# Kangfei/NNGP-src

Hardware: AMD Instinct MI355X
Metric: NNGP kernel-build + GP-solve wall-clock (ms) and GFLOP/s at N train queries (higher is better)
Workload: dtype f32 (Cholesky products as split f16 x3, f32 accumulate; f64 build/CG/means; the posterior's float64-grade residual as exact int8 digit-plane products); 1 GPU; synthetic N=32768, d=128, 5-layer ReLU NNGP + full Cholesky posterior (configs[2], north-star target); N=32768, d=128, n_relu=3, get=nngp, M_test=1024, parallelism=single GPU

## Files before the change

nngp-src_amd/csrc/api.hip:

```cpp
#include "model.h"

namespace nngp {

static thread_local char g_err[1024] = "";

void set_error(const char* fmt, ...) {
    va_list ap;
    va_start(ap, fmt);
    vsnprintf(g_err, sizeof(g_err), fmt, ap);
    va_end(ap);
}

int make_arch_dev(const nngp_arch* arch, ArchDev* out) {
    NNGP_REQUIRE(arch != nullptr, "arch is NULL");
    NNGP_REQUIRE(arch->n_dense >= 1 && arch->n_dense <= NNGP_MAX_DENSE, "arch.n_dense must be in [1, %d] (got %d)",
                 NNGP_MAX_DENSE, arch->n_dense);
    out->n_dense = arch->n_dense;
    out->groups = nullptr;
    for (int l = 0; l < NNGP_MAX_DENSE; ++l) {
        out->w2[l] = l < arch->n_dense ? arch->w_std[l] * arch->w_std[l] : 0.0;
        out->b2[l] = l < arch->n_dense ? arch->b_std[l] * arch->b_std[l] : 0.0;
    }
    return 0;
}
// ... 376 lines not shown
    NNGP_HIP_CHECK(hipStreamSynchronize(s));
    m->trace_mean = m->pcg.host_scal[7] / (double)n;
    m->diag_max = m->pcg.host_scal[6];
    m->reg = m->absolute ? m->diag_reg : m->diag_reg * m->trace_mean;
    m->reg_fac = m->reg;
    set_split_scale(m);
    m->have_train = true;
    return 0;
}

int nngp_model_build_rows(nngp_model* m, int64_t row_begin, int64_t row_end, void* stream) {
    hipStream_t s = (hipStream_t)stream;
    NNGP_REQUIRE(m != nullptr && m->have_train, "build_rows: call set_train first");
    NNGP_REQUIRE(0 <= row_begin && row_begin <= row_end && row_end <= m->n, "build_rows: bad row range");
    NNGP_TRY(drop_pending_solve(m));
    BuildArgs a{};
    a.x1 = m->x; a.x2 = m->x; a.q1 = m->q; a.q2 = m->q;
    a.n1 = m->n; a.n2 = m->n; a.d = m->d;
    a.row_begin = row_begin; a.row_end = row_end;
    a.sym = (row_begin == 0 && row_end == m->n) ? 1 : 0;
    a.ld64 = a.ld32 = m->ld;
    if (m->get == NNGP_GET_NNGP) a.nngp64 = m->k64; else a.ntk64 = m->k64;
    m->a32_built = false;
    m->a32_complete = false;
    m->k64_partial = false;
    m->k64_symmetric = a.sym != 0;
    m->i8.k.ready = false;
    m->i8_checked = m->i8_distrusted = false;
    m->i8_guard_pending = false;
    if (a.sym) {
// ... 10 lines not shown
        NNGP_TRY(launch_zero_pad_f64(m->kaux64, m->np, m->n, m->np, s));
        m->aux_ready = true;
        m->i8.aux.ready = false;
    }
    NNGP_TRY(launch_zero_pad_f64(m->k64, m->ld, m->n, m->np, s));
    m->built = true;
    m->factored = m->solved = false;
    m->solve_pending = false;
    return 0;
}

int nngp_model_factor_begin(nngp_model* m, void* stream) {
    hipStream_t s = (hipStream_t)stream;
    NNGP_REQUIRE(m != nullptr && m->built, "factor: build the kernel rows first");
    NNGP_TRY(drop_pending_solve(m));
    NNGP_TRY(launch_factor_input(m->k64, m->ld, m->a32, m->ld, m->n, m->np, m->reg_fac, m->reg_fac + m->trace_mean, s,
                                 m->a32_complete ? m->n : m->a32_built ? (m->n / TB) * TB : 0));
    m->a32_built = false;
    m->a32_complete = false;
    NNGP_HIP_CHECK(hipMemsetAsync(m->clamped, 0, sizeof(int32_t), s));
    m->tri.bs = triinv_block(m->np);
    m->factored = m->solved = false;
    m->solve_pending = false;
    m->serving_ready = false;
    m->split.l_ready = m->split.lt_ready = false;
    m->split.split_panel = -1;
    return 0;
}

int nngp_model_factor_panel(nngp_model* m, int64_t col0, int64_t width, void* stream) {
// ... 8 lines not shown
    return potrf_update_f32(m->a32, m->np, m->ld, panel_col0, panel_width, col0, width, (hipStream_t)stream, &m->split);
}

int nngp_model_factor_update_cols(nngp_model* m, int64_t panel_col0, int64_t panel_width, const int64_t* cols, int32_t ncols,
                                  int64_t width, void* stream) {
    NNGP_REQUIRE(m != nullptr && m->built, "factor_update_cols: build the kernel rows first");
    NNGP_REQUIRE(ncols >= 0 && (ncols == 0 || cols != nullptr), "factor_update_cols: bad column list");
    return potrf_update_cols_f32(m->a32, m->np, m->ld, panel_col0, panel_width, cols, ncols, width, (hipStream_t)stream, &m->split);
}

int nngp_model_factor_input_rows(nngp_model* m, int64_t row_begin, int64_t row_end, double shift_scale, void* stream) {
    hipStream_t s = (hipStream_t)stream;
    NNGP_REQUIRE(m != nullptr && m->built, "factor_input_rows: build the kernel rows first");
    NNGP_REQUIRE(0 <= row_begin && row_begin <= row_end && row_end <= m->n && shift_scale >= 1.0, "factor_input_rows: bad row range or shift");
    NNGP_TRY(drop_pending_solve(m));
    m->reg_fac = m->reg * shift_scale;
    m->k64_partial = true;
    return launch_factor_input(m->k64, m->ld, m->a32, m->ld, m->n, m->np, m->reg_fac, m->reg_fac + m->trace_mean, s, row_begin, row_end);
}

int nngp_model_factor_input_complete(nngp_model* m) {
    NNGP_REQUIRE(m != nullptr && m->built, "factor_input_complete: build the kernel rows first");
    NNGP_REQUIRE(m->k64_partial, "factor_input_complete: no rows of the factor input were converted (nngp_model_factor_input_rows) since the last build");
    m->a32_complete = true;
    return 0;
}

int nngp_model_precond(nngp_model* m, const double* r, double* z, void* stream) {
    NNGP_REQUIRE(m != nullptr && m->factored, "precond: factor first");
    NNGP_REQUIRE(r != nullptr && z != nullptr, "precond: NULL argument");
// ... 52 lines not shown
int nngp_model_factor(nngp_model* m, void* stream) {
    hipStream_t s = (hipStream_t)stream;
    NNGP_REQUIRE(m != nullptr && m->built, "factor: build the kernel rows first");
    if (!m->k64_partial) m->reg_fac = m->reg;
    set_split_scale(m);
    for (int attempt = 0;; ++attempt) {
        NNGP_TRY(nngp_model_factor_begin(m, stream));
        NNGP_TRY(potrf_lookahead_f32(m->a32, m->np, m->ld, m->dinv, m->clamped, (float)(0.25 * m->reg_fac), m->la, &m->split, s, &m->tri));
        int32_t cl = 0;
        NNGP_HIP_CHECK(hipMemcpyAsync(&cl, m->clamped, sizeof(int32_t), hipMemcpyDeviceToHost, s));
        NNGP_HIP_CHECK(hipStreamSynchronize(s));
        if (cl == 0 || attempt == 4 || NNGP_KNOB(6) == 1 || m->k64_partial) break;
        m->reg_fac *= 16.0;
        set_split_scale(m);
    }
    return nngp_model_factor_end(m, stream);
}

double nngp_model_factor_shift(nngp_model* m) { return m != nullptr ? m->reg_fac : 0.0; }

int nngp_model_append(nngp_model* m, const double* x_new, const double* y_new, int64_t b, void* stream) {
    hipStream_t s = (hipStream_t)stream;
    NNGP_REQUIRE(m != nullptr && m->factored, "append: fit the model first");
    NNGP_REQUIRE(!m->k64_partial, "append: not with the row-sharded layout (the model holds only its own kernel rows)");
    NNGP_REQUIRE(x_new != nullptr && y_new != nullptr && b > 0, "append: bad arguments");
    NNGP_REQUIRE(m->n + b <= m->n_cap, "append: %lld + %lld rows exceed n_cap = %lld", (long long)m->n, (long long)b,
                 (long long)m->n_cap);
    const int64_t n0 = m->n, n1 = n0 + b, np0 = m->np, np1 = round_up(n1, TB), r0 = (n0 / TB) * TB, rows = np1 - r0;
    NNGP_REQUIRE(r0 > 0, "append: the fitted model must have at least 128 rows");
    NNGP_TRY(drop_pending_solve(m));
    NNGP_TRY(ensure_predict_capacity(m, rows, false));
// ... 328 lines not shown
```

nngp-src_amd/csrc/api_predict.hip:

```cpp
#include "model.h"

namespace nngp {

int ensure_predict_capacity(nngp_model* m, int64_t mt, bool need_ktd) {
    if (mt > m->m_cap || m->b32 == nullptr) {
        const int64_t cap = mt > m->m_cap ? mt : m->m_cap;
        NNGP_HIP_CHECK(hipDeviceSynchronize());
        dev_free(m->xt_q); dev_free(m->tt_diag); dev_free(m->b32); dev_free(m->trsm_tmp);
        NNGP_TRY(dev_alloc(&m->xt_q, cap));
        NNGP_TRY(dev_alloc(&m->tt_diag, cap));
        NNGP_TRY(dev_alloc(&m->b32, round_up(cap, TB) * m->np_cap));
        NNGP_TRY(dev_alloc(&m->trsm_tmp, round_up(cap, TB) * triinv_block(m->np_cap)));
        if (m->split.planes != nullptr) {
            dev_free(m->split.planes_b); dev_free(m->split.row_inv);
            m->split.planes_b = nullptr; m->split.row_inv = nullptr;
            m->split.mb_cap = round_up(cap, TB);
            m->split.b_panels = (int)((triinv_block(m->np_cap) + m->split.k_cap - 1) / m->split.k_cap);
            NNGP_TRY(dev_alloc(&m->split.planes_b, (int64_t)(m->split.b_panels - 1) * m->split.col_stride + (m->split.mb_cap + 256) * m->split.k_cap * 4));
            NNGP_TRY(dev_alloc(&m->split.row_inv, m->split.mb_cap));
            tk_destroy(m->tk);
            m->tk = nullptr;
            if (m->split.k_cap == 1024 && triinv_block(m->np_cap) == 1024) NNGP_TRY(tk_create(&m->tk, m->np_cap, m->split.mb_cap) < 0 ? -1 : 0);
        }
        m->m_cap = cap;
// ... 169 lines not shown
int i8s_cut_planes(nngp_model* m, I8Planes& pk, const double* kmat, int64_t kld, hipStream_t s) {
    I8Work& w = m->i8;
    NNGP_TRY(launch_i8s_diag_bound_scale(kmat, kld, m->np, pk.scale, s));
    const bool sym = (kmat == m->kaux64 || m->k64_symmetric) && (pk.alloc_planes == 5 || pk.alloc_planes == 7) && NNGP_KNOB(5) != 62;
    if (sym)
        NNGP_TRY(launch_i8s_slice_sym(kmat, kld, m->np, pk.alloc_planes, pk.scale, pk.planes, m->np_cap, w.k_rows * m->np_cap, s));
    else
        NNGP_TRY(launch_i8s_slice_rows(kmat, kld, m->np, m->np, pk.alloc_planes, pk.scale, nullptr, pk.planes, m->np_cap, w.k_rows * m->np_cap, s));
    NNGP_TRY(launch_i8s_scale_sqsum(pk.scale, m->np, pk.scale + m->np_cap, s));
    pk.ns_done = pk.alloc_planes;
    pk.ready = true;
    return 0;
}

int i8s_product_rows(nngp_model* m, I8Planes& pk, const double* kmat, int64_t kld, double* out, const double* cin, double beta,
                     double alpha, double* z, double gamma, int64_t mp, hipStream_t s, int grade) {
    const int64_t np = m->np;
    I8Work& w = m->i8;
    const int fine_z = NNGP_KNOB(5) == 64 ? kI8FinePlanes : kI8FineZPlanes;
    const bool round_z = grade == I8_COARSE ? w.ns_z < w.ns_k : fine_z < kI8FinePlanes;
    const bool fuse_rows = grade == I8_COARSE && m->i8_fuse_request && cin != nullptr && w.rowpart_rows >= mp && NNGP_KNOB(5) != 59;
    const int ns_z = grade == I8_FINE ? fine_z : w.ns_z, ns_k = grade == I8_FINE ? kI8FinePlanes : w.ns_k;
    const int cut = grade == I8_FINE ? kI8FineCut : w.cut;
    NNGP_REQUIRE(pk.alloc_planes >= ns_k && w.z_planes >= ns_z, "i8s_product_rows: workspace for %d planes missing", ns_k);
    if (!pk.ready || pk.ns_done < ns_k) {
        NNGP_TRY(i8s_cut_planes(m, pk, kmat, kld, s));
    } else if (&pk == &m->i8.k && m->i8_k_pending) {
        NNGP_HIP_CHECK(hipStreamWaitEvent(s, m->ev_i8, 0));
    }
    if (&pk == &m->i8.k) m->i8_k_pending = false;
    I8Plan pl;
    NNGP_TRY(i8s_plan(ns_z, ns_k, cut, &pl));
    const int64_t nchunk = i8s_chunks(np, &pl);
    for (int64_t r0 = 0; r0 < mp; r0 += kI8RowBlock) {
        const int64_t mb = mp - r0 < kI8RowBlock ? mp - r0 : kI8RowBlock;
        const int64_t slab = mb * np;
        NNGP_TRY(launch_i8s_slice_rows(z + r0 * np, np, mb, np, ns_z, nullptr, w.zscale, w.zplanes, m->np_cap, (w.z_rows + 256) * m->np_cap, s,
                                       round_z ? z + r0 * np : nullptr));
        if (r0 == 0 && grade == I8_COARSE && !m->gate_recorded && NNGP_KNOB(2) != 8 && NNGP_KNOB(2) != 9 && !cg_from_the_start(m, mp)) {
            if (m->ev_gate == nullptr) NNGP_HIP_CHECK(hipEventCreateWithFlags(&m->ev_gate, hipEventDisableTiming));
            NNGP_HIP_CHECK(hipEventRecord(m->ev_gate, s));
            m->gate_recorded = true;
        }
        const bool timed = w.timed && w.t_count < I8Work::kMaxTimed;
        if (timed) {
            const int t = w.t_count;
            if (w.t0[t] == nullptr) NNGP_HIP_CHECK(hipEventCreate(&w.t0[t]));
            if (w.t1[t] == nullptr) NNGP_HIP_CHECK(hipEventCreate(&w.t1[t]));
            NNGP_HIP_CHECK(hipEventRecord(w.t0[t], s));
        }
        NNGP_TRY(launch_gemm_nt_i8s(w.partial, np, slab, w.zplanes, m->np_cap, (w.z_rows + 256) * m->np_cap, pk.planes, m->np_cap,
                                    w.k_rows * m->np_cap, pl, mb, np, np, w.counters, 0, s));
        if (timed) {
// ... 6 lines not shown
        fuse.out32 = m->b32 + r0 * np;
        fuse.ld32 = np;
        fuse.part = w.rowpart + r0 * i8s_col_blocks(np) * 4;
        NNGP_TRY(launch_i8s_combine(out + r0 * np, np, cin ? cin + r0 * np : nullptr, np, beta, alpha, z + r0 * np, np, gamma, w.partial, np,
                                    slab, (int)nchunk, pl.ndiag, w.zscale, pk.scale, mb, np, s, fuse_rows ? &fuse : nullptr));
    }
    if (fuse_rows) m->i8_fuse_done = true;
    if (grade == I8_COARSE && !m->gate_recorded && NNGP_KNOB(2) == 9) {
        if (m->ev_gate == nullptr) NNGP_HIP_CHECK(hipEventCreateWithFlags(&m->ev_gate, hipEventDisableTiming));
        NNGP_HIP_CHECK(hipEventRecord(m->ev_gate, s));
        m->gate_recorded = true;
    }
    return 0;
}

int residual_rows(nngp_model* m, double* out, const double* rhs, double* z, int64_t mp, hipStream_t s, bool first_residual) {
    const int64_t np = m->np;
    const bool coarse = first_residual;
    if (!coarse && use_i8s_fine(m, mp)) m->i8_want_fine = true;
    if (coarse ? use_i8s(m, mp) : use_i8s_fine(m, mp)) {
        const int rc = ensure_i8s(m, mp, m->i8.k, coarse ? i8s_planes_policy(m) : kI8FinePlanes);
        if (rc == 0) {
            if (coarse) m->i8_used_now = true;
            return i8s_product_rows(m, m->i8.k, m->k64, m->ld, out, rhs, 1.0, -1.0, z, -m->reg, mp, s, coarse ? I8_COARSE : I8_FINE);
        }
        if (rc != 1) return rc;
    }
    NNGP_TRY(launch_gemm_nt_f64(out, np, rhs, np, z, np, m->k64, m->ld, mp, np, np, -1.0, 1.0, s));
    return launch_axpby_mat(out, 1.0, z, -m->reg, np, mp, np, s);
}

int tri_join(nngp_model* m, hipStream_t s) {
    if (m->tri_stale) {
        if (m->ev_tri == nullptr) NNGP_HIP_CHECK(hipEventCreateWithFlags(&m->ev_tri, hipEventDisableTiming));
        NNGP_TRY(triinv_build(m->a32, m->ld, m->dinv, m->np, m->tri, s));
        if (m->tk != nullptr && m->tri.bs == 1024) NNGP_TRY(tk_prepare_inverses(m->tk, m->tri, m->np, m->a32, m->ld, s));
        NNGP_HIP_CHECK(hipEventRecord(m->ev_tri, s));
        m->tri_stale = false;
        m->tri_pending = true;
        return 0;
    }
    if (m->tri_pending) NNGP_HIP_CHECK(hipStreamWaitEvent(s, m->ev_tri, 0));
    if (m->tk != nullptr && !tk_inverses_ready(m->tk) && m->tri.bs == 1024) {
        NNGP_TRY(tk_prepare_inverses(m->tk, m->tri, m->np, m->a32, m->ld, s));
        if (m->ev_tri == nullptr) NNGP_HIP_CHECK(hipEventCreateWithFlags(&m->ev_tri, hipEventDisableTiming));
        NNGP_HIP_CHECK(hipEventRecord(m->ev_tri, s));
        m->tri_pending = true;
    }
    return 0;
}

int tri_fork(nngp_model* m, hipStream_t s) {
    if (!m->tri_stale || m->la == nullptr || m->la->panel == nullptr || NNGP_KNOB(5) == 61) return 0;
    if (m->ev_tri == nullptr) NNGP_HIP_CHECK(hipEventCreateWithFlags(&m->ev_tri, hipEventDisableTiming));
    if (m->ev_tri_fork == nullptr) NNGP_HIP_CHECK(hipEventCreateWithFlags(&m->ev_tri_fork, hipEventDisableTiming));
    NNGP_HIP_CHECK(hipEventRecord(m->ev_tri_fork, s));
    NNGP_HIP_CHECK(hipStreamWaitEvent(m->la->panel, m->ev_tri_fork, 0));
    NNGP_TRY(triinv_build(m->a32, m->ld, m->dinv, m->np, m->tri, m->la->panel));
    if (m->tk != nullptr && m->tri.bs == 1024) NNGP_TRY(tk_prepare_inverses(m->tk, m->tri, m->np, m->a32, m->ld, m->la->panel));
    NNGP_HIP_CHECK(hipEventRecord(m->ev_tri, m->la->panel));
    m->tri_stale = false;
    m->tri_pending = true;
    return 0;
}

bool use_split_solves(const nngp_model* m, int64_t mp) {
    return m->split.l_ready && m->split.planes_b != nullptr && mp <= m->split.mb_cap && m->tri.bs % m->split.k_cap == 0 &&
           m->tri.bs / m->split.k_cap <= m->split.b_panels && m->tri.bs <= 2048 && NNGP_KNOB(7) == 0 && mp >= 256 && mp * m->np >= 7000000;
}

bool use_tickets(const nngp_model* m, int64_t mp) {
    return !m->tk_failed && m->tri.bs == 1024 && tk_usable(m->tk, mp, m->np) && NNGP_KNOB(9) != 16;
}

bool cg_from_the_start(const nngp_model* m, int64_t mp) {
    static const int env = getenv("NNGP_TK_GATE") ? atoi(getenv("NNGP_TK_GATE")) : 1;
    return env != 0 && use_split_solves(m, mp) && use_tickets(m, mp);
// ... 77 lines not shown
    else NNGP_TRY(ensure_lt(m, s));
    int slot = -1;
    NNGP_TRY(trsm_timer_begin(m, mp, s, &slot));
    if (use_split_solves(m, mp) && use_tickets(m, mp))
        NNGP_TRY(tk_solve(m->tk, m->b32, m->np, mp, m->np, m->split, true, s, tickets_reserve(m)));
    else if (use_split_solves(m, mp))
        NNGP_TRY(trsm_rut_blocks_h3(m->b32, m->np, mp, m->lt_ready ? m->lt32 : nullptr, m->np, m->tri, m->np, m->trsm_tmp, m->split, s));
    else
        NNGP_TRY(trsm_rut_blocks_f32(m->b32, m->np, mp, m->lt32, m->np, m->tri, m->np, m->trsm_tmp, s));
    return trsm_timer_end(m, slot, s);
}

static int ntk_sweeps(const nngp_model* m) { return m->var_refine < 2 ? 2 : m->var_refine; }

int refined_solve_rows(nngp_model* m, const double* rhs, int64_t mp, int sweeps, bool final_residual, hipStream_t s,
                       bool measure) {
    const int64_t np = m->np;
    measure = measure && sweeps >= 2;
    NNGP_TRY(launch_convert_f64_f32(rhs, np, m->b32, np, mp, np, mp, np, s));
    NNGP_TRY(apply_inverse_f32(m, mp, s));
    NNGP_TRY(launch_f32_to_f64_mat(m->b32, np, m->z64, np, mp, np, false, s));
    for (int it = 0; it < sweeps + (final_residual ? 1 : 0); ++it) {
        NNGP_TRY(residual_rows(m, m->r64, rhs, m->z64, mp, s, it == 0));
        if (it == sweeps) break;
        NNGP_TRY(launch_convert_f64_f32(m->r64, np, m->b32, np, mp, np, mp, np, s));
        NNGP_TRY(apply_inverse_f32(m, mp, s));
        if (measure && it < 2) NNGP_TRY(launch_rows_energy(m->r64, m->b32, np, mp, np, it == 0 ? m->rows.var : m->rows.delta, s));
        NNGP_TRY(launch_f32_to_f64_mat(m->b32, np, m->z64, np, mp, np, true, s));
    }
    if (measure) NNGP_TRY(launch_rowdot_f64(m->z64, nullptr, 0.0, rhs, np, mp, np, nullptr, 1.0, m->rows.tol, s));
    return 0;
}

int rows_pcg_continue(nngp_model* m, int64_t mp, int max_iters, hipStream_t s) {
    const int64_t np = m->np;
    RowsPcg& w = m->rows;
    if (mp > m->rows_pq_cap) {
        NNGP_HIP_CHECK(hipDeviceSynchronize());
// ... 9 lines not shown
        NNGP_TRY(apply_inverse_f32(m, mp, s));
        NNGP_TRY(launch_rows_rho(m->r64, m->b32, np, mp, np, it == 0, w, s));
        NNGP_TRY(launch_rows_update_p(w.p, m->b32, np, mp, np, w, s));
        NNGP_TRY(launch_gemm_nt_f64(w.q, np, w.p, np, w.p, np, m->k64, m->ld, mp, np, np, 1.0, m->reg, s));
        NNGP_TRY(launch_rows_alpha(w.p, w.q, np, mp, np, w, s));
        NNGP_TRY(launch_rows_axpy2(m->z64, m->r64, w.p, w.q, np, mp, np, w, s));
        NNGP_HIP_CHECK(hipMemcpyAsync(w.host, w.live, sizeof(int32_t), hipMemcpyDeviceToHost, s));
        NNGP_HIP_CHECK(hipStreamSynchronize(s));
        m->cov_iters = it + 1;
        if (w.host[0] == 0) break;
    }
    return 0;
}

int build_cross(nngp_model* m, const double* xt, const double* qt, int64_t mt, int64_t mp, bool nngp, double* out,
                hipStream_t s) {
    NNGP_HIP_CHECK(hipMemsetAsync(out, 0, sizeof(double) * mp * m->np, s));
    BuildArgs a{};
    a.x1 = xt; a.x2 = m->x; a.q1 = qt; a.q2 = m->q;
    a.n1 = mt; a.n2 = m->n; a.d = m->d;
    a.row_begin = 0; a.row_end = mt; a.sym = 0;
    a.ld64 = a.ld32 = m->np;
    if (nngp) a.nngp64 = out; else a.ntk64 = out;
    return launch_kernel_build(a, m->arch, s);
}

}

extern "C" {

int nngp_model_prepare_serving(nngp_model* m, void* stream) {
    hipStream_t s = (hipStream_t)stream;
    NNGP_REQUIRE(m != nullptr && m->solved, "prepare_serving: fit the model first");
    NNGP_REQUIRE(!m->k64_partial, "prepare_serving: not with the row-sharded layout (the model holds only its own kernel rows)");
    if (m->get != NNGP_GET_NNGP) return 0;
    NNGP_TRY(run_pending_solve(m, s, true));
    const int64_t n = m->n, np = m->np;
    const int64_t blk = np < 1024 ? np : 1024;
// ... 61 lines not shown
            static const int cut_env = getenv("NNGP_TK_CUTSTREAM") ? atoi(getenv("NNGP_TK_CUTSTREAM")) : 2;
            hipStream_t cs = m->solve_stream;
            if (cut_env != 0 && cg_from_the_start(m, mp) && m->la != nullptr && m->la->panel != nullptr)
                cs = (cut_env == 2 && m->la->update != nullptr) ? m->la->update : m->la->panel;
            NNGP_HIP_CHECK(hipStreamWaitEvent(cs, m->ev_i8, 0));
            NNGP_TRY(i8s_cut_planes(m, m->i8.k, m->k64, m->ld, cs));
            NNGP_HIP_CHECK(hipEventRecord(m->ev_i8, cs));
            m->i8_k_pending = true;
        }
    }
    NNGP_TRY(tri_fork(m, s));

    const double* xt = on_train ? m->x : x_test;
    const double* ktd = m->k64;
    const double* qt = m->q;
    if (!on_train) {
        NNGP_TRY(launch_row_sqnorm(xt, mt, m->d, m->xt_q, s));
        qt = m->xt_q;
        NNGP_TRY(build_cross(m, xt, qt, mt, mp, !is_ntk, m->ktd64, s));
        ktd = m->ktd64;
    }
    if (compact_train) {
        NNGP_HIP_CHECK(hipMemsetAsync(m->ktd64, 0, sizeof(double) * mp * np, s));
        NNGP_HIP_CHECK(hipMemcpy2DAsync(m->ktd64, sizeof(double) * np, m->k64, sizeof(double) * m->ld, sizeof(double) * np, mt,
                                        hipMemcpyDeviceToDevice, s));
        ktd = m->ktd64;
    }
    if (m->i8_guard_pending && hipEventQuery(m->ev_guard) == hipSuccess) {
        double ratio = 0.0;
        memcpy(&ratio, m->i8_guard_host, sizeof(double));
        m->i8_guard_pending = false;
        if (ratio > m->i8_floor_ratio) m->i8_floor_ratio = ratio;
        if (!(ratio <= (NNGP_KNOB(5) == 56 ? 0.0 : kI8FloorThr))) m->i8_distrusted = true;
    }
    int check_kind = 0;
    bool i8_check_pending = false;
// ... 21 lines not shown
    const double kFlagThr = (NNGP_KNOB(6) >= 2 && NNGP_KNOB(6) <= 30) ? pow(10.0, -(double)NNGP_KNOB(6)) : 1e-8;
    auto cov_part = [&]() -> int {
    if (full) NNGP_TRY(ensure_full_cov_capacity(m, mt));
    NNGP_TRY(launch_kernel_diag(xt, qt, mt, m->d, m->arch, m->tt_diag, nullptr, s));
    auto build_ktt = [&]() -> int {
        BuildArgs a{};
        a.x1 = xt; a.x2 = xt; a.q1 = qt; a.q2 = qt;
        a.n1 = mt; a.n2 = mt; a.d = m->d;
        a.row_begin = 0; a.row_end = mt; a.sym = 1;
        a.ld64 = a.ld32 = mp;
        a.nngp64 = m->ktt64;
        return launch_kernel_build(a, m->arch, s);
    };

    if (!is_ntk && m->var_refine == 0) {
        NNGP_TRY(launch_convert_f64_f32(ktd, np, m->b32, np, mp, np, mp, np, s));
        NNGP_TRY(apply_forward_f32(m, mp, s));
        if (!full) return launch_row_sqsum_f32(m->b32, np, mt, np, m->tt_diag, var_or_cov, s);
        NNGP_TRY(build_ktt());
        NNGP_TRY(launch_gemm_nt_f32(m->vvt32, mp, m->b32, np, m->b32, np, mp, mp, np, 1.0f, 0.0f, false, s));
        return launch_cov_finish(m->ktt64, mp, m->vvt32, mp, mt, var_or_cov, s);
    }

    const bool serving = m->serving_ready && !is_ntk;
    if (!serving && !use_split_solves(m, mp)) NNGP_TRY(ensure_lt(m, s));
    NNGP_TRY(ensure_refine_capacity(m, mp));
    auto solve_rows = [&](int sweeps, bool final_residual) -> int {
        if (!serving) return refined_solve_rows(m, ktd, mp, sweeps, final_residual, s);
        NNGP_TRY(launch_gemm_nt_f64(m->z64, np, nullptr, 0, ktd, np, m->ainv64, np, mp, np, np, 1.0, 0.0, s));
        if (m->serving_weak) {
            NNGP_TRY(residual_rows(m, m->r64, ktd, m->z64, mp, s, false));
            NNGP_TRY(launch_gemm_nt_f64(m->z64, np, m->z64, np, m->r64, np, m->ainv64, np, mp, np, np, 1.0, 1.0, s));
        }
        if (final_residual) {
            NNGP_TRY(residual_rows(m, m->r64, ktd, m->z64, mp, s, false));
        }
        return 0;
    };
    if (!is_ntk) {
        const int level = ((serving || (full && m->var_refine == 1)) && m->var_refine < 2) ? 2 : m->var_refine;
        const bool second_order = level >= 2;
        if (!full && level == 1) {
            m->i8_fuse_request = true;
// ... 94 lines not shown
        NNGP_TRY(launch_zero_pad_f64(m->kaux64, np, n, np, s));
        m->aux_ready = true;
        m->i8.aux.ready = false;
    }
    const double* ktd_n = m->kaux64;
    if (!on_train) {
        if (mp > m->ktd_aux_cap) {
            NNGP_HIP_CHECK(hipDeviceSynchronize());
            dev_free(m->ktd_aux);
            NNGP_TRY(dev_alloc(&m->ktd_aux, mp * m->np_cap));
            m->ktd_aux_cap = mp;
        }
        NNGP_TRY(build_cross(m, xt, qt, mt, mp, true, m->ktd_aux, s));
        ktd_n = m->ktd_aux;
    }
    NNGP_TRY(refined_solve_rows(m, ktd, mp, ntk_sweeps(m), false, s, m->var_refine >= 1));
    ntk_cross = ktd_n;
    z_valid = true;
    if (full) NNGP_TRY(build_ktt());
    if (m->var_refine >= 1) check_kind = 3;
    NNGP_TRY(ntk_finish());
    if (check_kind == 3) {
        NNGP_TRY(launch_rows_dvar(m->b32, m->r64, full ? nullptr : ntk_cross, -1.0, np, mt, np, m->rows.coef, s));
        NNGP_TRY(launch_sweep_estimate(m->rows.var, m->rows.delta, m->rows.tol, m->rows.coef, var_or_cov, full ? mt + 1 : 1,
                                       mt, reinterpret_cast<double*>(m->rows.live + 2), s));
    }
    return 0;
    };
    if (cov_mode != NNGP_COV_NONE) NNGP_TRY(cov_part());
    NNGP_TRY(run_pending_solve(m, s, true, z_valid));
    if (i8_check_pending) {
// ... 81 lines not shown
```

nngp-src_amd/csrc/common.h:

```cpp
#pragma once
#include <hip/hip_runtime.h>
#include <stdint.h>
#include <atomic>
#include <stdio.h>
#include <string.h>

#include "../../include/nngp_hip.h"
#include "../../include/nngp_rbf_gp.h"
#include "../../include/nngp_activations.h"
#include "../../include/nngp_mll.h"
#include "../../include/nngp_additive.h"
#include "../../include/nngp_pool.h"
#include "../../include/nngp_sparse.h"

namespace nngp {

constexpr int TB = 128;

void set_error(const char* fmt, ...);
void note_alloc();
#ifdef NNGP_TIMING_KNOBS
extern std::atomic<int> g_knobs[16];
#define NNGP_KNOB(i) (nngp::g_knobs[i].load(std::memory_order_relaxed))
#else
// ... 209 lines not shown
    hipEvent_t t0[kMaxTimed] = {}, t1[kMaxTimed] = {};
    int t_count = 0;
    double t_ops[kMaxTimed] = {};
    double t_flops[kMaxTimed] = {};
};
int i8s_plan(int nsa, int nsb, int cut, I8Plan* pl);
int64_t i8s_chunks(int64_t k, const I8Plan* pl = nullptr);
int launch_i8s_diag_bound_scale(const double* src, int64_t ld, int64_t n, double* scale, hipStream_t s);
int launch_i8s_scale_sqsum(const double* scale, int64_t n, double* out, hipStream_t s);
int launch_i8s_floor_ratio(const double* z, int64_t ld, int64_t rows, int64_t cols, const double* var, const I8Plan& pl, int nsa, int nsb,
                           const double* sk2, unsigned long long* out, hipStream_t s);
int launch_i8s_floor_ratio_rows(const double* zstat, int64_t rows, const double* var, const I8Plan& pl, int nsa, int nsb, const double* sk2,
                                unsigned long long* out, hipStream_t s);
int launch_i8s_slice_rows(const double* src, int64_t ld, int64_t rows, int64_t cols, int ns, const double* scale_in, double* scale_out,
                          int8_t* planes, int64_t ldp, int64_t pstride, hipStream_t s, double* writeback = nullptr);
int launch_i8s_slice_sym(const double* src, int64_t ld, int64_t n, int ns, const double* scale, int8_t* planes, int64_t ldp,
                         int64_t pstride, hipStream_t s);
int launch_gemm_nt_i8s(int32_t* partial, int64_t ldc, int64_t slab, const int8_t* a, int64_t lda, int64_t sa, const int8_t* b,
                       int64_t ldb, int64_t sb, const I8Plan& pl, int64_t m, int64_t n, int64_t k, int* counters, int reserve_cus,
                       hipStream_t s);
struct I8Fuse {
    float* out32 = nullptr;
    int64_t ld32 = 0;
    double* part = nullptr;
};
int64_t i8s_col_blocks(int64_t cols);
int launch_i8s_combine(double* out, int64_t ldo, const double* cin, int64_t ldcin, double beta, double alpha, const double* g,
                       int64_t ldg, double gamma, const int32_t* partial, int64_t ldc, int64_t slab, int nchunk, int ndiag,
                       const double* sa, const double* sb, int64_t rows, int64_t cols, hipStream_t s, const I8Fuse* fuse = nullptr);
int launch_i8s_rowstat_finish(const double* part, int64_t cols, int64_t rows, const double* base, double* var, double* delta,
// ... 133 lines not shown
```

nngp-src_amd/csrc/gemm_i8s.hip:

```cpp
#include <atomic>

#include "common.h"

namespace nngp {

namespace {

typedef int i32x4 __attribute__((ext_vector_type(4)));
typedef double f64x2 __attribute__((ext_vector_type(2)));
typedef __attribute__((address_space(3))) void lds_void;
typedef const __attribute__((address_space(1))) void glb_void;

constexpr int IT = 256;
constexpr int IROW = 128;
constexpr int ISTAGE = 2 * IT * IROW;
constexpr int kI8ChunkBlocks = 128;
constexpr int kI8ChunkBlocks3 = 320;

__device__ __forceinline__ double i8s_scale_of(double mx) {
    if (!(mx > 0.0 && mx < 1.0e300)) return 1.0;
    int e = 0;
    const double f = frexp(mx, &e);
    return ldexp(1.0, f <= 0.984375 ? e + 1 : e + 2);
}
// ... 3 lines not shown
    __shared__ double red[16];
    double mx = 0.0;
    for (int64_t i = threadIdx.x; i < n; i += 1024) mx = fmax(mx, fabs(src[i * ld + i]));
#pragma unroll
    for (int off = 32; off > 0; off >>= 1) mx = fmax(mx, __shfl_xor(mx, off));
    if ((threadIdx.x & 63) == 0) red[threadIdx.x >> 6] = mx;
    __syncthreads();
    mx = 0.0;
#pragma unroll
    for (int i = 0; i < 16; ++i) mx = fmax(mx, red[i]);
    for (int64_t i = threadIdx.x; i < n; i += 1024) {
        scale[i] = i8s_scale_of(sqrt(fabs(src[i * ld + i]) * mx) * (1.0 + 1e-9));
    }
}

template <int NS>
__global__ __launch_bounds__(256) void k_i8s_slice_rows(const double* src, int64_t ld, int64_t cols, int64_t kp,
                                                        const double* __restrict__ scale_in, double* __restrict__ scale_out,
                                                        int8_t* __restrict__ planes, int64_t ldp, int64_t pstride, double* wb) {
    __shared__ __attribute__((aligned(16))) unsigned char dig[NS][4096];
    __shared__ double red[4];
    const int t = threadIdx.x;
    const int64_t r = blockIdx.x;
    const double* p = src + r * ld;
    double scale;
    if (scale_in != nullptr) {
        scale = scale_in[r];
    } else {
        double mx = 0.0;
        for (int64_t c = 2 * (int64_t)t; c < cols; c += 512) {
            if (c + 1 < cols) {
                const f64x2 v = *reinterpret_cast<const f64x2*>(p + c);
                mx = fmax(mx, fmax(fabs(v[0]), fabs(v[1])));
            } else {
                mx = fmax(mx, fabs(p[c]));
            }
        }
#pragma unroll
        for (int off = 32; off > 0; off >>= 1) mx = fmax(mx, __shfl_xor(mx, off));
        if ((t & 63) == 0) red[t >> 6] = mx;
        __syncthreads();
        scale = i8s_scale_of(fmax(fmax(red[0], red[1]), fmax(red[2], red[3])));
        if (t == 0) scale_out[r] = scale;
    }
    const double inv = ldexp(1.0, 8 * NS) / scale;
    const double back = scale * ldexp(1.0, -8 * NS);
    double* q = wb != nullptr ? wb + r * ld : nullptr;
    for (int64_t seg0 = 0; seg0 < kp; seg0 += 4096) {
#pragma unroll
        for (int i = 0; i < 8; ++i) {
            const int lc = 2 * t + 512 * i;
            const int64_t c = seg0 + lc;
            f64x2 v = {0.0, 0.0};
            if (c + 1 < cols) {
                v = *reinterpret_cast<const f64x2*>(p + c);
            } else if (c < cols) {
                v[0] = p[c];
            }
            long long x0 = __double2ll_rn(v[0] * inv), x1 = __double2ll_rn(v[1] * inv);
            if (q != nullptr) {
                if (c + 1 < cols) {
                    *reinterpret_cast<f64x2*>(q + c) = f64x2{(double)x0 * back, (double)x1 * back};
                } else if (c < cols) {
                    q[c] = (double)x0 * back;
                }
            }
#pragma unroll
            for (int s = NS - 1; s >= 1; --s) {
                const long long d0 = ((x0 + 128) & 255) - 128, d1 = ((x1 + 128) & 255) - 128;
                x0 = (x0 - d0) >> 8;
                x1 = (x1 - d1) >> 8;
                *reinterpret_cast<unsigned short*>(&dig[s][lc]) = (unsigned short)((d0 & 255) | ((d1 & 255) << 8));
// ... 451 lines not shown
    const double est = sqrt(zstat[2 * r]) * coef * i8s_scale_of(zstat[2 * r + 1]) * sqrt(sk2[0]);
    const double v = var[r];
    const double ratio = v > 0.0 ? est / v : (est > 0.0 ? 1.0e300 : 0.0);
    atomicMax(out, (unsigned long long)__double_as_longlong(ratio));
}

}

int launch_i8s_diag_bound_scale(const double* src, int64_t ld, int64_t n, double* scale, hipStream_t s) {
    if (n <= 0) return 0;
    hipLaunchKernelGGL(k_i8s_diag_bound_scale, dim3(1), dim3(1024), 0, s, src, ld, n, scale);
    NNGP_HIP_CHECK(hipGetLastError());
    return 0;
}

int launch_i8s_slice_rows(const double* src, int64_t ld, int64_t rows, int64_t cols, int ns, const double* scale_in, double* scale_out,
                          int8_t* planes, int64_t ldp, int64_t pstride, hipStream_t s, double* writeback) {
    if (rows <= 0) return 0;
    const int64_t kp = round_up(cols, 128);
    NNGP_REQUIRE(ns >= 2 && ns <= 7 && ld % 2 == 0 && ((uintptr_t)src & 15) == 0 && ((uintptr_t)planes & 15) == 0 && ldp >= kp &&
                     ldp % 16 == 0 && pstride % 16 == 0 && rows < 2147483647LL && (scale_in != nullptr || scale_out != nullptr),
                 "i8s_slice_rows: 2..7 planes, 16-byte aligned operands");
    const dim3 g((unsigned)rows);
    switch (ns) {
        case 2: hipLaunchKernelGGL(k_i8s_slice_rows<2>, g, dim3(256), 0, s, src, ld, cols, kp, scale_in, scale_out, planes, ldp, pstride, writeback); break;
        case 3: hipLaunchKernelGGL(k_i8s_slice_rows<3>, g, dim3(256), 0, s, src, ld, cols, kp, scale_in, scale_out, planes, ldp, pstride, writeback); break;
        case 4: hipLaunchKernelGGL(k_i8s_slice_rows<4>, g, dim3(256), 0, s, src, ld, cols, kp, scale_in, scale_out, planes, ldp, pstride, writeback); break;
        case 5: hipLaunchKernelGGL(k_i8s_slice_rows<5>, g, dim3(256), 0, s, src, ld, cols, kp, scale_in, scale_out, planes, ldp, pstride, writeback); break;
        case 6: hipLaunchKernelGGL(k_i8s_slice_rows<6>, g, dim3(256), 0, s, src, ld, cols, kp, scale_in, scale_out, planes, ldp, pstride, writeback); break;
        default: hipLaunchKernelGGL(k_i8s_slice_rows<7>, g, dim3(256), 0, s, src, ld, cols, kp, scale_in, scale_out, planes, ldp, pstride, writeback); break;
    }
    NNGP_HIP_CHECK(hipGetLastError());
    return 0;
}

int launch_i8s_slice_sym(const double* src, int64_t ld, int64_t n, int ns, const double* scale, int8_t* planes, int64_t ldp,
                         int64_t pstride, hipStream_t s) {
    if (n <= 0) return 0;
    NNGP_REQUIRE((ns == 5 || ns == 7) && n % kSymT == 0 && ld % 2 == 0 && ((uintptr_t)src & 15) == 0 && ((uintptr_t)planes & 15) == 0 &&
                     ldp >= n && ldp % 16 == 0 && pstride % 16 == 0 && scale != nullptr,
                 "i8s_slice_sym: 5 or 7 planes of a matrix padded to 128");
    const int64_t tn = n / kSymT, tiles = tn * (tn + 1) / 2;
    NNGP_REQUIRE(tiles < 2147483647LL, "i8s_slice_sym: too many tiles");
    if (ns == 5) hipLaunchKernelGGL(k_i8s_slice_sym<5>, dim3((unsigned)tiles), dim3(256), 0, s, src, ld, scale, planes, ldp, pstride);
    else hipLaunchKernelGGL(k_i8s_slice_sym<7>, dim3((unsigned)tiles), dim3(256), 0, s, src, ld, scale, planes, ldp, pstride);
    NNGP_HIP_CHECK(hipGetLastError());
    return 0;
}
// ... 160 lines not shown
```

nngp-src_amd/csrc/model.h:

```cpp
#pragma once
#include <stdarg.h>
#include <stdlib.h>
#include <cmath>
#include <new>
#include <mutex>
#include "common.h"
#include <atomic>

namespace nngp {
extern std::atomic<long long> g_alloc_count;

template <typename T>
inline int dev_alloc(T** p, int64_t count) {
    *p = nullptr;
    if (count <= 0) return 0;
    NNGP_HIP_CHECK(hipMalloc(reinterpret_cast<void**>(p), sizeof(T) * (size_t)count));
    g_alloc_count.fetch_add(1, std::memory_order_relaxed);
    return 0;
}

template <typename T>
inline void dev_free(T*& p) {
    if (p) (void)hipFree(p);
    p = nullptr;
// ... 159 lines not shown
namespace nngp {
int ensure_predict_capacity(nngp_model* m, int64_t mt, bool need_ktd);
int ensure_full_cov_capacity(nngp_model* m, int64_t mt);
int drop_pending_solve(nngp_model* m);
void set_split_scale(nngp_model* m);
int ensure_refine_capacity(nngp_model* m, int64_t mp);
int ensure_lt_alloc(nngp_model* m);
int ensure_lt(nngp_model* m, hipStream_t s);
int ensure_lt_split(nngp_model* m, hipStream_t s);
bool use_i8s(const nngp_model* m, int64_t mp);
bool use_i8s_fine(const nngp_model* m, int64_t mp);
int i8s_planes_policy(const nngp_model* m);
int ensure_i8s(nngp_model* m, int64_t mp, I8Planes& pk, int planes);
int i8s_cut_planes(nngp_model* m, I8Planes& pk, const double* kmat, int64_t kld, hipStream_t s);
int i8s_product_rows(nngp_model* m, I8Planes& pk, const double* kmat, int64_t kld, double* out, const double* cin, double beta,
                     double alpha, double* z, double gamma, int64_t mp, hipStream_t s, int grade);
int residual_rows(nngp_model* m, double* out, const double* rhs, double* z, int64_t mp, hipStream_t s, bool first_residual);
int tri_join(nngp_model* m, hipStream_t s);
int tri_fork(nngp_model* m, hipStream_t s);
bool use_split_solves(const nngp_model* m, int64_t mp);
bool use_tickets(const nngp_model* m, int64_t mp);
bool cg_from_the_start(const nngp_model* m, int64_t mp);
int tickets_reserve(const nngp_model* m);
int tickets_check(nngp_model* m, bool wait);
int apply_forward_f32(nngp_model* m, int64_t mp, hipStream_t s);
int apply_inverse_f32(nngp_model* m, int64_t mp, hipStream_t s);
int refined_solve_rows(nngp_model* m, const double* rhs, int64_t mp, int sweeps, bool final_residual, hipStream_t s,
                       bool measure = false);
int rows_pcg_continue(nngp_model* m, int64_t mp, int max_iters, hipStream_t s);
int build_cross(nngp_model* m, const double* xt, const double* qt, int64_t mt, int64_t mp, bool nngp, double* out,
                hipStream_t s);
int run_pending_solve(nngp_model* m, hipStream_t user, bool order_user, bool allow_partial = false);
}
```

Before: 172,600 GFLOP/s.

## Fuse f32 cross-kernel and z slicing into build and slice kernels; fork triangular inverses after factor

The cross-kernel build now also writes the f32 right-hand side directly, so the separate f64-to-f32 conversion is skipped. The first coarse residual slices z straight from the f32 solve output into int8 planes and writes back the rounded f64 copy in the same kernel, removing one f32-to-f64 conversion pass. The first z slab is cut before the K planes to reorder work. Triangular-inverse construction is forked onto the panel stream right after factorization so it overlaps with later work, and tri_settle guards later writes to a32. This adds cross-stream ordering complexity and more memset traffic for the extra f32 buffer.

```diff
diff --git a/nngp-src_amd/csrc/api.hip b/nngp-src_amd/csrc/api.hip
--- a/nngp-src_amd/csrc/api.hip
+++ b/nngp-src_amd/csrc/api.hip
@@ -414,6 +414,7 @@
     NNGP_REQUIRE(m != nullptr && m->have_train, "build_rows: call set_train first");
     NNGP_REQUIRE(0 <= row_begin && row_begin <= row_end && row_end <= m->n, "build_rows: bad row range");
     NNGP_TRY(drop_pending_solve(m));
+    NNGP_TRY(tri_settle(m, s));
     BuildArgs a{};
     a.x1 = m->x; a.x2 = m->x; a.q1 = m->q; a.q2 = m->q;
     a.n1 = m->n; a.n2 = m->n; a.d = m->d;
@@ -454,6 +455,7 @@
     hipStream_t s = (hipStream_t)stream;
     NNGP_REQUIRE(m != nullptr && m->built, "factor: build the kernel rows first");
     NNGP_TRY(drop_pending_solve(m));
+    NNGP_TRY(tri_settle(m, s));
     NNGP_TRY(launch_factor_input(m->k64, m->ld, m->a32, m->ld, m->n, m->np, m->reg_fac, m->reg_fac + m->trace_mean, s,
                                  m->a32_complete ? m->n : m->a32_built ? (m->n / TB) * TB : 0));
     m->a32_built = false;
@@ -492,6 +494,7 @@
     NNGP_REQUIRE(m != nullptr && m->built, "factor_input_rows: build the kernel rows first");
     NNGP_REQUIRE(0 <= row_begin && row_begin <= row_end && row_end <= m->n && shift_scale >= 1.0, "factor_input_rows: bad row range or shift");
     NNGP_TRY(drop_pending_solve(m));
+    NNGP_TRY(tri_settle(m, s));
     m->reg_fac = m->reg * shift_scale;
     m->k64_partial = true;
     return launch_factor_input(m->k64, m->ld, m->a32, m->ld, m->n, m->np, m->reg_fac, m->reg_fac + m->trace_mean, s, row_begin, row_end);
@@ -574,7 +577,9 @@
         m->reg_fac *= 16.0;
         set_split_scale(m);
     }
-    return nngp_model_factor_end(m, stream);
+    NNGP_TRY(nngp_model_factor_end(m, stream));
+    if (NNGP_KNOB(5) != 69) NNGP_TRY(tri_fork(m, s));
+    return 0;
 }
 
 double nngp_model_factor_shift(nngp_model* m) { return m != nullptr ? m->reg_fac : 0.0; }
diff --git a/nngp-src_amd/csrc/api_predict.hip b/nngp-src_amd/csrc/api_predict.hip
--- a/nngp-src_amd/csrc/api_predict.hip
+++ b/nngp-src_amd/csrc/api_predict.hip
@@ -207,7 +207,7 @@
 }
 
 int i8s_product_rows(nngp_model* m, I8Planes& pk, const double* kmat, int64_t kld, double* out, const double* cin, double beta,
-                     double alpha, double* z, double gamma, int64_t mp, hipStream_t s, int grade) {
+                     double alpha, double* z, double gamma, int64_t mp, hipStream_t s, int grade, const float* z32) {
     const int64_t np = m->np;
     I8Work& w = m->i8;
     const int fine_z = NNGP_KNOB(5) == 64 ? kI8FinePlanes : kI8FineZPlanes;
@@ -216,6 +216,16 @@
     const int ns_z = grade == I8_FINE ? fine_z : w.ns_z, ns_k = grade == I8_FINE ? kI8FinePlanes : w.ns_k;
     const int cut = grade == I8_FINE ? kI8FineCut : w.cut;
     NNGP_REQUIRE(pk.alloc_planes >= ns_k && w.z_planes >= ns_z, "i8s_product_rows: workspace for %d planes missing", ns_k);
+    NNGP_REQUIRE(z32 == nullptr || (grade == I8_COARSE && round_z), "i8s_product_rows: float32 rows only where z is rounded and written back");
+    auto cut_z = [&](int64_t r0, int64_t mb) -> int {
+        if (z32 != nullptr)
+            return launch_i8s_slice_rows_f32(z32 + r0 * np, np, mb, np, ns_z, w.zscale, w.zplanes, m->np_cap, (w.z_rows + 256) * m->np_cap, s,
+                                             z + r0 * np);
+        return launch_i8s_slice_rows(z + r0 * np, np, mb, np, ns_z, nullptr, w.zscale, w.zplanes, m->np_cap, (w.z_rows + 256) * m->np_cap, s,
+                                     round_z ? z + r0 * np : nullptr);
+    };
+    const bool z_first = NNGP_KNOB(5) != 67;
+    if (z_first) NNGP_TRY(cut_z(0, mp < kI8RowBlock ? mp : kI8RowBlock));
     if (!pk.ready || pk.ns_done < ns_k) {
         NNGP_TRY(i8s_cut_planes(m, pk, kmat, kld, s));
     } else if (&pk == &m->i8.k && m->i8_k_pending) {
@@ -228,8 +238,7 @@
     for (int64_t r0 = 0; r0 < mp; r0 += kI8RowBlock) {
         const int64_t mb = mp - r0 < kI8RowBlock ? mp - r0 : kI8RowBlock;
         const int64_t slab = mb * np;
-        NNGP_TRY(launch_i8s_slice_rows(z + r0 * np, np, mb, np, ns_z, nullptr, w.zscale, w.zplanes, m->np_cap, (w.z_rows + 256) * m->np_cap, s,
-                                       round_z ? z + r0 * np : nullptr));
+        if (r0 > 0 || !z_first) NNGP_TRY(cut_z(r0, mb));
         if (r0 == 0 && grade == I8_COARSE && !m->gate_recorded && NNGP_KNOB(2) != 8 && NNGP_KNOB(2) != 9 && !cg_from_the_start(m, mp)) {
             if (m->ev_gate == nullptr) NNGP_HIP_CHECK(hipEventCreateWithFlags(&m->ev_gate, hipEventDisableTiming));
             NNGP_HIP_CHECK(hipEventRecord(m->ev_gate, s));
@@ -266,7 +275,8 @@
     return 0;
 }
 
-int residual_rows(nngp_model* m, double* out, const double* rhs, double* z, int64_t mp, hipStream_t s, bool first_residual) {
+int residual_rows(nngp_model* m, double* out, const double* rhs, double* z, int64_t mp, hipStream_t s, bool first_residual,
+                  const float* z32) {
     const int64_t np = m->np;
     const bool coarse = first_residual;
     if (!coarse && use_i8s_fine(m, mp)) m->i8_want_fine = true;
@@ -274,10 +284,14 @@
         const int rc = ensure_i8s(m, mp, m->i8.k, coarse ? i8s_planes_policy(m) : kI8FinePlanes);
         if (rc == 0) {
             if (coarse) m->i8_used_now = true;
-            return i8s_product_rows(m, m->i8.k, m->k64, m->ld, out, rhs, 1.0, -1.0, z, -m->reg, mp, s, coarse ? I8_COARSE : I8_FINE);
+            const bool fused_z = z32 != nullptr && coarse && m->i8.ns_z < m->i8.ns_k;
+            if (z32 != nullptr && !fused_z) NNGP_TRY(launch_f32_to_f64_mat(z32, np, z, np, mp, np, false, s));
+            return i8s_product_rows(m, m->i8.k, m->k64, m->ld, out, rhs, 1.0, -1.0, z, -m->reg, mp, s, coarse ? I8_COARSE : I8_FINE,
+                                    fused_z ? z32 : nullptr);
         }
         if (rc != 1) return rc;
     }
+    if (z32 != nullptr) NNGP_TRY(launch_f32_to_f64_mat(z32, np, z, np, mp, np, false, s));
     NNGP_TRY(launch_gemm_nt_f64(out, np, rhs, np, z, np, m->k64, m->ld, mp, np, np, -1.0, 1.0, s));
     return launch_axpby_mat(out, 1.0, z, -m->reg, np, mp, np, s);
 }
@@ -303,16 +317,24 @@
 }
 
 int tri_fork(nngp_model* m, hipStream_t s) {
-    if (!m->tri_stale || m->la == nullptr || m->la->panel == nullptr || NNGP_KNOB(5) == 61) return 0;
+    if (m->la == nullptr || m->la->panel == nullptr || NNGP_KNOB(5) == 61) return 0;
+    const bool tk_missing = m->tk != nullptr && m->tri.bs == 1024 && !tk_inverses_ready(m->tk);
+    if (!m->tri_stale && !tk_missing) return 0;
     if (m->ev_tri == nullptr) NNGP_HIP_CHECK(hipEventCreateWithFlags(&m->ev_tri, hipEventDisableTiming));
     if (m->ev_tri_fork == nullptr) NNGP_HIP_CHECK(hipEventCreateWithFlags(&m->ev_tri_fork, hipEventDisableTiming));
     NNGP_HIP_CHECK(hipEventRecord(m->ev_tri_fork, s));
     NNGP_HIP_CHECK(hipStreamWaitEvent(m->la->panel, m->ev_tri_fork, 0));
-    NNGP_TRY(triinv_build(m->a32, m->ld, m->dinv, m->np, m->tri, m->la->panel));
+    if (m->tri_stale) NNGP_TRY(triinv_build(m->a32, m->ld, m->dinv, m->np, m->tri, m->la->panel));
+    else if (m->tri_pending) NNGP_HIP_CHECK(hipStreamWaitEvent(m->la->panel, m->ev_tri, 0));
     if (m->tk != nullptr && m->tri.bs == 1024) NNGP_TRY(tk_prepare_inverses(m->tk, m->tri, m->np, m->a32, m->ld, m->la->panel));
     NNGP_HIP_CHECK(hipEventRecord(m->ev_tri, m->la->panel));
     m->tri_stale = false;
     m->tri_pending = true;
+    return 0;
+}
+
+int tri_settle(nngp_model* m, hipStream_t s) {
+    if (!m->tri_stale && m->tri_pending) NNGP_HIP_CHECK(hipStreamWaitEvent(s, m->ev_tri, 0));
     return 0;
 }
 
@@ -420,14 +442,15 @@
 static int ntk_sweeps(const nngp_model* m) { return m->var_refine < 2 ? 2 : m->var_refine; }
 
 int refined_solve_rows(nngp_model* m, const double* rhs, int64_t mp, int sweeps, bool final_residual, hipStream_t s,
-                       bool measure) {
+                       bool measure, bool rhs_in_b32) {
     const int64_t np = m->np;
     measure = measure && sweeps >= 2;
-    NNGP_TRY(launch_convert_f64_f32(rhs, np, m->b32, np, mp, np, mp, np, s));
+    if (!rhs_in_b32) NNGP_TRY(launch_convert_f64_f32(rhs, np, m->b32, np, mp, np, mp, np, s));
     NNGP_TRY(apply_inverse_f32(m, mp, s));
-    NNGP_TRY(launch_f32_to_f64_mat(m->b32, np, m->z64, np, mp, np, false, s));
+    const bool z_pending = sweeps + (final_residual ? 1 : 0) > 0 && NNGP_KNOB(5) != 67;
+    if (!z_pending) NNGP_TRY(launch_f32_to_f64_mat(m->b32, np, m->z64, np, mp, np, false, s));
     for (int it = 0; it < sweeps + (final_residual ? 1 : 0); ++it) {
-        NNGP_TRY(residual_rows(m, m->r64, rhs, m->z64, mp, s, it == 0));
+        NNGP_TRY(residual_rows(m, m->r64, rhs, m->z64, mp, s, it == 0, (it == 0 && z_pending) ? m->b32 : nullptr));
         if (it == sweeps) break;
         NNGP_TRY(launch_convert_f64_f32(m->r64, np, m->b32, np, mp, np, mp, np, s));
         NNGP_TRY(apply_inverse_f32(m, mp, s));
@@ -467,14 +490,15 @@
 }
 
 int build_cross(nngp_model* m, const double* xt, const double* qt, int64_t mt, int64_t mp, bool nngp, double* out,
-                hipStream_t s) {
+                hipStream_t s, float* out32) {
     NNGP_HIP_CHECK(hipMemsetAsync(out, 0, sizeof(double) * mp * m->np, s));
+    if (out32 != nullptr) NNGP_HIP_CHECK(hipMemsetAsync(out32, 0, sizeof(float) * mp * m->np, s));
     BuildArgs a{};
     a.x1 = xt; a.x2 = m->x; a.q1 = qt; a.q2 = m->q;
     a.n1 = mt; a.n2 = m->n; a.d = m->d;
     a.row_begin = 0; a.row_end = mt; a.sym = 0;
     a.ld64 = a.ld32 = m->np;
-    if (nngp) a.nngp64 = out; else a.ntk64 = out;
+    if (nngp) { a.nngp64 = out; a.nngp32 = out32; } else { a.ntk64 = out; a.ntk32 = out32; }
     return launch_kernel_build(a, m->arch, s);
 }
 
@@ -566,12 +590,15 @@
     const double* xt = on_train ? m->x : x_test;
     const double* ktd = m->k64;
     const double* qt = m->q;
+    bool rhs32_ready = false;
     if (!on_train) {
         NNGP_TRY(launch_row_sqnorm(xt, mt, m->d, m->xt_q, s));
         qt = m->xt_q;
-        NNGP_TRY(build_cross(m, xt, qt, mt, mp, !is_ntk, m->ktd64, s));
+        rhs32_ready = cov_mode != NNGP_COV_NONE && !(m->serving_ready && !is_ntk) && NNGP_KNOB(5) != 68;
+        NNGP_TRY(build_cross(m, xt, qt, mt, mp, !is_ntk, m->ktd64, s, rhs32_ready ? m->b32 : nullptr));
         ktd = m->ktd64;
     }
+    auto take_rhs32 = [&]() -> bool { const bool r = rhs32_ready; rhs32_ready = false; return r; };
     if (compact_train) {
         NNGP_HIP_CHECK(hipMemsetAsync(m->ktd64, 0, sizeof(double) * mp * np, s));
         NNGP_HIP_CHECK(hipMemcpy2DAsync(m->ktd64, sizeof(double) * np, m->k64, sizeof(double) * m->ld, sizeof(double) * np, mt,
@@ -623,7 +650,7 @@
     };
 
     if (!is_ntk && m->var_refine == 0) {
-        NNGP_TRY(launch_convert_f64_f32(ktd, np, m->b32, np, mp, np, mp, np, s));
+        if (!take_rhs32()) NNGP_TRY(launch_convert_f64_f32(ktd, np, m->b32, np, mp, np, mp, np, s));
         NNGP_TRY(apply_forward_f32(m, mp, s));
         if (!full) return launch_row_sqsum_f32(m->b32, np, mt, np, m->tt_diag, var_or_cov, s);
         NNGP_TRY(build_ktt());
@@ -635,7 +662,7 @@
     if (!serving && !use_split_solves(m, mp)) NNGP_TRY(ensure_lt(m, s));
     NNGP_TRY(ensure_refine_capacity(m, mp));
     auto solve_rows = [&](int sweeps, bool final_residual) -> int {
-        if (!serving) return refined_solve_rows(m, ktd, mp, sweeps, final_residual, s);
+        if (!serving) return refined_solve_rows(m, ktd, mp, sweeps, final_residual, s, false, take_rhs32());
         NNGP_TRY(launch_gemm_nt_f64(m->z64, np, nullptr, 0, ktd, np, m->ainv64, np, mp, np, np, 1.0, 0.0, s));
         if (m->serving_weak) {
             NNGP_TRY(residual_rows(m, m->r64, ktd, m->z64, mp, s, false));
@@ -760,7 +787,7 @@
         NNGP_TRY(build_cross(m, xt, qt, mt, mp, true, m->ktd_aux, s));
         ktd_n = m->ktd_aux;
     }
-    NNGP_TRY(refined_solve_rows(m, ktd, mp, ntk_sweeps(m), false, s, m->var_refine >= 1));
+    NNGP_TRY(refined_solve_rows(m, ktd, mp, ntk_sweeps(m), false, s, m->var_refine >= 1, take_rhs32()));
     ntk_cross = ktd_n;
     z_valid = true;
     if (full) NNGP_TRY(build_ktt());
diff --git a/nngp-src_amd/csrc/common.h b/nngp-src_amd/csrc/common.h
--- a/nngp-src_amd/csrc/common.h
+++ b/nngp-src_amd/csrc/common.h
@@ -247,6 +247,8 @@
                                 unsigned long long* out, hipStream_t s);
 int launch_i8s_slice_rows(const double* src, int64_t ld, int64_t rows, int64_t cols, int ns, const double* scale_in, double* scale_out,
                           int8_t* planes, int64_t ldp, int64_t pstride, hipStream_t s, double* writeback = nullptr);
+int launch_i8s_slice_rows_f32(const float* src, int64_t ld, int64_t rows, int64_t cols, int ns, double* scale_out, int8_t* planes,
+                              int64_t ldp, int64_t pstride, hipStream_t s, double* writeback);
 int launch_i8s_slice_sym(const double* src, int64_t ld, int64_t n, int ns, const double* scale, int8_t* planes, int64_t ldp,
                          int64_t pstride, hipStream_t s);
 int launch_gemm_nt_i8s(int32_t* partial, int64_t ldc, int64_t slab, const int8_t* a, int64_t lda, int64_t sa, const int8_t* b,
diff --git a/nngp-src_amd/csrc/gemm_i8s.hip b/nngp-src_amd/csrc/gemm_i8s.hip
--- a/nngp-src_amd/csrc/gemm_i8s.hip
+++ b/nngp-src_amd/csrc/gemm_i8s.hip
@@ -8,6 +8,7 @@
 
 typedef int i32x4 __attribute__((ext_vector_type(4)));
 typedef double f64x2 __attribute__((ext_vector_type(2)));
+typedef float f32x2 __attribute__((ext_vector_type(2)));
 typedef __attribute__((address_space(3))) void lds_void;
 typedef const __attribute__((address_space(1))) void glb_void;
 
@@ -41,15 +42,19 @@
     }
 }
 
-template <int NS>
-__global__ __launch_bounds__(256) void k_i8s_slice_rows(const double* src, int64_t ld, int64_t cols, int64_t kp,
+template <typename T> struct I8Pair;
+template <> struct I8Pair<double> { typedef f64x2 type; };
+template <> struct I8Pair<float> { typedef f32x2 type; };
+template <int NS, typename T>
+__global__ __launch_bounds__(256) void k_i8s_slice_rows(const T* src, int64_t ld, int64_t cols, int64_t kp,
                                                         const double* __restrict__ scale_in, double* __restrict__ scale_out,
                                                         int8_t* __restrict__ planes, int64_t ldp, int64_t pstride, double* wb) {
+    typedef typename I8Pair<T>::type pair_t;
     __shared__ __attribute__((aligned(16))) unsigned char dig[NS][4096];
     __shared__ double red[4];
     const int t = threadIdx.x;
     const int64_t r = blockIdx.x;
-    const double* p = src + r * ld;
+    const T* p = src + r * ld;
     double scale;
     if (scale_in != nullptr) {
         scale = scale_in[r];
@@ -57,10 +62,10 @@
         double mx = 0.0;
         for (int64_t c = 2 * (int64_t)t; c < cols; c += 512) {
             if (c + 1 < cols) {
-                const f64x2 v = *reinterpret_cast<const f64x2*>(p + c);
-                mx = fmax(mx, fmax(fabs(v[0]), fabs(v[1])));
+                const pair_t v = *reinterpret_cast<const pair_t*>(p + c);
+                mx = fmax(mx, fmax(fabs((double)v[0]), fabs((double)v[1])));
             } else {
-                mx = fmax(mx, fabs(p[c]));
+                mx = fmax(mx, fabs((double)p[c]));
             }
         }
 #pragma unroll
@@ -80,9 +85,10 @@
             const int64_t c = seg0 + lc;
             f64x2 v = {0.0, 0.0};
             if (c + 1 < cols) {
-                v = *reinterpret_cast<const f64x2*>(p + c);
+                const pair_t w = *reinterpret_cast<const pair_t*>(p + c);
+                v = f64x2{(double)w[0], (double)w[1]};
             } else if (c < cols) {
-                v[0] = p[c];
+                v[0] = (double)p[c];
             }
             long long x0 = __double2ll_rn(v[0] * inv), x1 = __double2ll_rn(v[1] * inv);
             if (q != nullptr) {
@@ -564,24 +570,37 @@
     return 0;
 }
 
-int launch_i8s_slice_rows(const double* src, int64_t ld, int64_t rows, int64_t cols, int ns, const double* scale_in, double* scale_out,
-                          int8_t* planes, int64_t ldp, int64_t pstride, hipStream_t s, double* writeback) {
+template <typename T>
+static int i8s_slice_rows_any(const T* src, int64_t ld, int64_t rows, int64_t cols, int ns, const double* scale_in, double* scale_out,
+                              int8_t* planes, int64_t ldp, int64_t pstride, hipStream_t s, double* writeback) {
     if (rows <= 0) return 0;
     const int64_t kp = round_up(cols, 128);
-    NNGP_REQUIRE(ns >= 2 && ns <= 7 && ld % 2 == 0 && ((uintptr_t)src & 15) == 0 && ((uintptr_t)planes & 15) == 0 && ldp >= kp &&
-                     ldp % 16 == 0 && pstride % 16 == 0 && rows < 2147483647LL && (scale_in != nullptr || scale_out != nullptr),
+    NNGP_REQUIRE(ns >= 2 && ns <= 7 && ld % 2 == 0 && ((uintptr_t)src & (2 * sizeof(T) - 1)) == 0 && ((uintptr_t)planes & 15) == 0 && ldp >= kp &&
+                     ((uintptr_t)writeback & 15) == 0 && ldp % 16 == 0 && pstride % 16 == 0 && rows < 2147483647LL &&
+                     (scale_in != nullptr || scale_out != nullptr),
                  "i8s_slice_rows: 2..7 planes, 16-byte aligned operands");
     const dim3 g((unsigned)rows);
     switch (ns) {
-        case 2: hipLaunchKernelGGL(k_i8s_slice_rows<2>, g, dim3(256), 0, s, src, ld, cols, kp, scale_in, scale_out, planes, ldp, pstride, writeback); break;
-        case 3: hipLaunchKernelGGL(k_i8s_slice_rows<3>, g, dim3(256), 0, s, src, ld, cols, kp, scale_in, scale_out, planes, ldp, pstride, writeback); break;
-        case 4: hipLaunchKernelGGL(k_i8s_slice_rows<4>, g, dim3(256), 0, s, src, ld, cols, kp, scale_in, scale_out, planes, ldp, pstride, writeback); break;
-        case 5: hipLaunchKernelGGL(k_i8s_slice_rows<5>, g, dim3(256), 0, s, src, ld, cols, kp, scale_in, scale_out, planes, ldp, pstride, writeback); break;
-        case 6: hipLaunchKernelGGL(k_i8s_slice_rows<6>, g, dim3(256), 0, s, src, ld, cols, kp, scale_in, scale_out, planes, ldp, pstride, writeback); break;
-        default: hipLaunchKernelGGL(k_i8s_slice_rows<7>, g, dim3(256), 0, s, src, ld, cols, kp, scale_in, scale_out, planes, ldp, pstride, writeback); break;
-    }
-    NNGP_HIP_CHECK(hipGetLastError());
-    return 0;
+        case 2: hipLaunchKernelGGL((k_i8s_slice_rows<2, T>), g, dim3(256), 0, s, src, ld, cols, kp, scale_in, scale_out, planes, ldp, pstride, writeback); break;
+        case 3: hipLaunchKernelGGL((k_i8s_slice_rows<3, T>), g, dim3(256), 0, s, src, ld, cols, kp, scale_in, scale_out, planes, ldp, pstride, writeback); break;
+        case 4: hipLaunchKernelGGL((k_i8s_slice_rows<4, T>), g, dim3(256), 0, s, src, ld, cols, kp, scale_in, scale_out, planes, ldp, pstride, writeback); break;
+        case 5: hipLaunchKernelGGL((k_i8s_slice_rows<5, T>), g, dim3(256), 0, s, src, ld, cols, kp, scale_in, scale_out, planes, ldp, pstride, writeback); break;
+        case 6: hipLaunchKernelGGL((k_i8s_slice_rows<6, T>), g, dim3(256), 0, s, src, ld, cols, kp, scale_in, scale_out, planes, ldp, pstride, writeback); break;
+        default: hipLaunchKernelGGL((k_i8s_slice_rows<7, T>), g, dim3(256), 0, s, src, ld, cols, kp, scale_in, scale_out, planes, ldp, pstride, writeback); break;
+    }
+    NNGP_HIP_CHECK(hipGetLastError());
+    return 0;
+}
+
+int launch_i8s_slice_rows(const double* src, int64_t ld, int64_t rows, int64_t cols, int ns, const double* scale_in, double* scale_out,
+                          int8_t* planes, int64_t ldp, int64_t pstride, hipStream_t s, double* writeback) {
+    return i8s_slice_rows_any(src, ld, rows, cols, ns, scale_in, scale_out, planes, ldp, pstride, s, writeback);
+}
+
+int launch_i8s_slice_rows_f32(const float* src, int64_t ld, int64_t rows, int64_t cols, int ns, double* scale_out, int8_t* planes,
+                              int64_t ldp, int64_t pstride, hipStream_t s, double* writeback) {
+    NNGP_REQUIRE(writeback != nullptr && scale_out != nullptr, "i8s_slice_rows_f32: the rounded float64 rows need a destination");
+    return i8s_slice_rows_any(src, ld, rows, cols, ns, (const double*)nullptr, scale_out, planes, ldp, pstride, s, writeback);
 }
 
 int launch_i8s_slice_sym(const double* src, int64_t ld, int64_t n, int ns, const double* scale, int8_t* planes, int64_t ldp,
diff --git a/nngp-src_amd/csrc/model.h b/nngp-src_amd/csrc/model.h
--- a/nngp-src_amd/csrc/model.h
+++ b/nngp-src_amd/csrc/model.h
@@ -197,10 +197,12 @@
 int ensure_i8s(nngp_model* m, int64_t mp, I8Planes& pk, int planes);
 int i8s_cut_planes(nngp_model* m, I8Planes& pk, const double* kmat, int64_t kld, hipStream_t s);
 int i8s_product_rows(nngp_model* m, I8Planes& pk, const double* kmat, int64_t kld, double* out, const double* cin, double beta,
-                     double alpha, double* z, double gamma, int64_t mp, hipStream_t s, int grade);
-int residual_rows(nngp_model* m, double* out, const double* rhs, double* z, int64_t mp, hipStream_t s, bool first_residual);
+                     double alpha, double* z, double gamma, int64_t mp, hipStream_t s, int grade, const float* z32 = nullptr);
+int residual_rows(nngp_model* m, double* out, const double* rhs, double* z, int64_t mp, hipStream_t s, bool first_residual,
+                  const float* z32 = nullptr);
 int tri_join(nngp_model* m, hipStream_t s);
 int tri_fork(nngp_model* m, hipStream_t s);
+int tri_settle(nngp_model* m, hipStream_t s);
 bool use_split_solves(const nngp_model* m, int64_t mp);
 bool use_tickets(const nngp_model* m, int64_t mp);
 bool cg_from_the_start(const nngp_model* m, int64_t mp);
@@ -209,9 +211,9 @@
 int apply_forward_f32(nngp_model* m, int64_t mp, hipStream_t s);
 int apply_inverse_f32(nngp_model* m, int64_t mp, hipStream_t s);
 int refined_solve_rows(nngp_model* m, const double* rhs, int64_t mp, int sweeps, bool final_residual, hipStream_t s,
-                       bool measure = false);
+                       bool measure = false, bool rhs_in_b32 = false);
 int rows_pcg_continue(nngp_model* m, int64_t mp, int max_iters, hipStream_t s);
 int build_cross(nngp_model* m, const double* xt, const double* qt, int64_t mt, int64_t mp, bool nngp, double* out,
-                hipStream_t s);
+                hipStream_t s, float* out32 = nullptr);
 int run_pending_solve(nngp_model* m, hipStream_t user, bool order_user, bool allow_partial = false);
 }
```

After: 173,400 GFLOP/s (median of 6 runs). About the same (+0.4%).
